# david8862/tf-keras-deeplabv3p-model-set

Measured on AMD Instinct MI355X. Metric: images/sec (513x513, 21-class) MobileNetV2-DeepLabV3+ OS=16 training step, higher is better.
Workload: dtype f32

## Files before the change

### tf-keras-deeplabv3p-model-set_amd/csrc/options.h

```cpp
#pragma once
#include "common.h"

enum OptGet { GET_NONE, GET_SET, GET_LATCHED, GET_LATCHED_GE0, GET_RESOLVED };

#define DL3P_OPTION_TABLE(X)                                                                                                  \
                                                                    \
  X(PW_SMALL_MIN_ROWS, GET_NONE, "pw_small_min_rows", "DL3P_PW_SMALL_MIN_ROWS", 1 << 17, -1, v < 0 ? (1 << 17) : v)           \
                                \
  X(GEMM_NT, GET_NONE, "gemm_nt", nullptr, 0, 0, (v >= 1 && v <= 8) ? v : 0)                                                  \
              \
  X(GEMM_MI, GET_NONE, "gemm_mi", "DL3P_GEMM_MI", 0, 0, (v == 1 || v == 2) ? v : 0)                                           \
  X(GEMM_PER_CU, GET_NONE, "gemm_per_cu", "DL3P_GEMM_PER_CU", 0, 0, v > 0 ? v : 0)                                            \
                                                                \
  X(GEMM_TUNED, GET_NONE, "gemm_tuned", "DL3P_GEMM_TUNED", 1, -1, v ? 1 : 0)                                                  \
                   \
  X(SB_PIPE, GET_RESOLVED, "sb_pipe", "DL3P_SB_PIPE", 0, -1, v ? 1 : 0)                                                       \
                                                        \
  X(SPLIT_WGRAD, GET_LATCHED, "split_wgrad", "DL3P_SPLIT_WGRAD", env_int("DL3P_SPLIT_GEMM", 1), -1, v ? 1 : 0)                \
           \
  X(SPLIT_WGRAD_TILE, GET_NONE, "split_wgrad_tile", nullptr, -1, -1, (v >= 0 && v <= 4) ? v : -1)                             \
  X(SPLIT_WGRAD_PER_CU, GET_NONE, "split_wgrad_per_cu", nullptr, 0, 0, v > 0 ? v : 0)                                         \
                                                        \
  X(SPLITK, GET_SET, "splitk", "DL3P_SPLITK", -1, -1, v)                                                                      \
                     \
  X(SB_WM, GET_NONE, "sb_wm", nullptr, 0, 0, (v >= -1 && v <= 2) ? v : 0)                                                     \
  X(SB_NT, GET_NONE, "sb_nt", nullptr, 0, 0, (v == 8 || v == 12 || v == 16) ? v : 0)                                          \
                                       \
  X(SB_RS, GET_SET, "sb_rs", "DL3P_SB_RS", -1, -1, v < 0 ? -1 : (v ? 1 : 0))                                                  \
                                        \
  X(SB3, GET_LATCHED_GE0, "sb3", "DL3P_SB3", -1, -1, v < 0 ? -1 : (v ? 1 : 0))                                                \
                                     \
  X(BF16_KG, GET_NONE, "bf16_kg", "DL3P_BF16_KG", 0, -1, (v == 0 || v == 1 || v == 2 || v == 4) ? v : -1)                     \
                        \
  X(CONV_SB, GET_SET, "conv_sb", "DL3P_CONV_SB", 1, -1, (v >= 0 && v <= 2) ? v : -1)                                          \
                                      \
  X(DW_PER_CU, GET_NONE, "dw_per_cu", nullptr, 0, 0, v > 0 ? v : 0)                                                           \
  X(DW_WANT, GET_NONE, "dw_want", "DL3P_DW_WANT", DL3P_NUM_CUS * 3 / 2, 0, v > 0 ? v : 0)                                     \
  X(DW_MAXTH, GET_NONE, "dw_maxth", "DL3P_DW_MAXTH", 16, 0, v > 0 ? v : 0)                                                    \
  X(DW_TW, GET_NONE, "dw_tw", nullptr, 0, 0, (v == 2 || v == 4) ? v : 0)                                                      \
  X(DW_TUNED, GET_NONE, "dw_tuned", "DL3P_DW_TUNED", 1, -1, v ? 1 : 0)                                                        \
                                                                                                               \
  X(WGRAD_TILE, GET_NONE, "wgrad_tile", "DL3P_WGRAD_TILE", -1, -1, (v >= 0 && v <= 3) ? v : -1)                               \
  X(WGRAD_PER_CU, GET_NONE, "wgrad_per_cu", "DL3P_WGRAD_PER_CU", 4, 0, v > 0 ? v : 0)

enum Opt {
#define X(id, get, name, env, def, unset, norm) OPT_##id,
  DL3P_OPTION_TABLE(X)
#undef X
  OPT_COUNT
};

struct OptState { int set, env; bool env_read; };
extern OptState g_opt[OPT_COUNT];
int opt_env_read(Opt id);

static constexpr int k_opt_unset[OPT_COUNT] = {
#define X(id, get, name, env, def, unset, norm) unset,
  DL3P_OPTION_TABLE(X)
#undef X
};

static inline int opt_set(Opt id) { return g_opt[id].set; }
static inline int opt_env(Opt id) { return g_opt[id].env_read ? g_opt[id].env : opt_env_read(id); }
static inline int opt(Opt id) { return g_opt[id].set != k_opt_unset[id] ? g_opt[id].set : opt_env(id); }
```

### tf-keras-deeplabv3p-model-set_amd/csrc/pw_gemm_kernels.h

```cpp
#pragma once
#include "pw_gemm.h"
#include <type_traits>

typedef float f32x4 __attribute__((ext_vector_type(4)));

#ifndef DL3P_GEMM_PIN_B
#define DL3P_GEMM_PIN_B 1
#endif
template <int NT, bool B_KN, bool STATS, int MI, int BKT, bool BNB = false, bool GA = false>
__global__ __launch_bounds__(256, 2) void pw_gemm_kernel(GemmParams p_in) {
  GemmParams p = p_in;
  int block_y = blockIdx.y;
#ifndef DL3P_NO_SPLITK
  if constexpr (!B_KN && !STATS && !BNB && !GA) {
    if (p.ksplit > 1) {
      const int nbn = (int)gridDim.y / p.ksplit;
      const int z = block_y / nbn;
      block_y -= z * nbn;
      const int k_lo = z * p.kchunk;
      p.A += k_lo;
      if (p.scale) { p.scale += k_lo; p.shift += k_lo; }
      p.B += k_lo;
      p.K = min(p.kchunk, p.K - k_lo);
      p.Y += (size_t)z * p.M * p.ldy;
// ... 353 lines not shown
    for (int idx = t; idx < KP * NP; idx += 256) {
      const int n = idx / KP, k = idx - n * KP;
      Bs[k * BP + n] = (k < p.K && n < p.N) ? p.B[(size_t)n * p.ldb + k] : 0.f;
    }
  }
  for (int i = t; i < KP; i += 256) {
    sc_s[i] = (p.scale && i < p.K) ? p.scale[i] : 1.f;
    sh_s[i] = (p.scale && i < p.K) ? p.shift[i] : 0.f;
  }
  if (BNB) {
    for (int i = t; i < NP; i += 256) {
      const bool in = i < p.N;
      bq_s[i] = in ? p.bb_scale[i] : 1.f;
      bq_s[NP + i] = in ? p.bb_shift[i] : 0.f;
      bq_s[2 * NP + i] = in ? p.bb_mean[i] : 0.f;
      bq_s[3 * NP + i] = in ? p.bb_invstd[i] : 0.f;
    }
  }
  __syncthreads();

  uint32_t a_k[KT];
  bool a_kok[KT];
#pragma unroll
  for (int kt = 0; kt < KT; ++kt) {
    const int k = kt * 16 + 4 * q;
    a_kok[kt] = k < p.K;
    a_k[kt] = (uint32_t)min(k, p.K - 4) * 4u;
  }
  const int n4 = p.N >> 2, nf = 4 * p.N;
  int yrow[NTN], yl[NTN];
  uint32_t yg[NTN], zg[BNB ? NTN : 1];
#pragma unroll
  for (int i = 0; i < NTN; ++i) {
    const int f = min(l + 64 * i, nf - 1);
    const int r = f / n4, c = f - r * n4;
    yrow[i] = (l + 64 * i < nf) ? r : (1 << 20);
    yl[i] = r * TP + c * 4;
    yg[i] = ((uint32_t)r * (uint32_t)p.ldy + (uint32_t)c * 4u) * 4u;
    if (BNB) zg[i] = ((uint32_t)r * (uint32_t)p.bb_ldz + (uint32_t)c * 4u) * 4u;
  }
  const char* Zb = reinterpret_cast<const char*>(p.bb_z);
  const float act_lo = p.act == DL3P_ACT_NONE ? -DL3P_INF : 0.f;
  const float act_hi = (p.act == DL3P_ACT_NONE || p.act == DL3P_ACT_RELU) ? DL3P_INF : 6.f;

  f32x4 acc[NTN];
#pragma unroll
  for (int b = 0; b < NTN; ++b) acc[b] = (f32x4){0.f, 0.f, 0.f, 0.f};
  float4 st_s[STATS ? NTN : 1], st_q[STATS ? NTN : 1];
  if (STATS) {
#pragma unroll
    for (int i = 0; i < NTN; ++i) { st_s[i] = zero4(); st_q[i] = zero4(); }
  }

  const int ntiles = (p.M + 15) >> 4;
  const int nwaves = gridDim.x * 4;
  const int gw = blockIdx.x * 4 + w;
  const char* Ab = reinterpret_cast<const char*>(p.A);
  char* Yb = reinterpret_cast<char*>(p.Y);
  float4 ra[KT];
#define SM_PREFETCH(tile_)                                                                                   \
  {                                                                                                          \
    const uint32_t arow = (uint32_t)min(((tile_) << 4) + l15, p.M - 1) * (uint32_t)p.lda * 4u;              \
    _Pragma("unroll") for (int kt = 0; kt < KT; ++kt) ra[kt] = *reinterpret_cast<const float4*>(Ab + (arow + a_k[kt])); \
  }
  SM_PREFETCH(min(gw, ntiles - 1))
  for (int tile = gw; tile < ntiles; tile += nwaves) {
    const int m0 = tile << 4;
    const bool row_ok = m0 + l15 < p.M;
    float4 zpre[BNB ? NTN : 1];
    if (BNB) {
      const uint32_t zbase = (uint32_t)m0 * (uint32_t)p.bb_ldz * 4u;
#pragma unroll
      for (int i = 0; i < NTN; ++i) {
        const uint32_t off = (yrow[i] < p.M - m0) ? zg[i] : 0u;
        zpre[i] = *reinterpret_cast<const float4*>(Zb + (zbase + off));
      }
    }
    float4 a[KT];
#pragma unroll
    for (int kt = 0; kt < KT; ++kt) {
      const float4 s4 = *reinterpret_cast<const float4*>(&sc_s[kt * 16 + 4 * q]);
      const float4 h4 = *reinterpret_cast<const float4*>(&sh_s[kt * 16 + 4 * q]);
      float4 v = fma4(ra[kt], s4, h4);
      if (p.act >= DL3P_ACT_HSWISH) v = act_apply4(v, p.act);
      else v = make_float4(__builtin_amdgcn_fmed3f(v.x, act_lo, act_hi), __builtin_amdgcn_fmed3f(v.y, act_lo, act_hi),
                           __builtin_amdgcn_fmed3f(v.z, act_lo, act_hi), __builtin_amdgcn_fmed3f(v.w, act_lo, act_hi));
      a[kt] = (row_ok && a_kok[kt]) ? v : zero4();
    }
    SM_PREFETCH(min(tile + nwaves, ntiles - 1))
#pragma unroll
    for (int kt = 0; kt < KT; ++kt) {
      const float av[4] = {a[kt].x, a[kt].y, a[kt].z, a[kt].w};
#pragma unroll
      for (int nt = 0; nt < NTN; ++nt)
#pragma unroll
        for (int j = 0; j < 4; ++j)
          acc[nt] = __builtin_amdgcn_mfma_f32_16x16x4f32(Bs[(kt * 16 + 4 * q + j) * BP + nt * 16 + l15], av[j], acc[nt], 0, 0, 0);
    }
#pragma unroll
    for (int nt = 0; nt < NTN; ++nt) {
      *reinterpret_cast<float4*>(&Ts[l15 * TP + nt * 16 + 4 * q]) = make_float4(acc[nt][0], acc[nt][1], acc[nt][2], acc[nt][3]);
      acc[nt] = (f32x4){0.f, 0.f, 0.f, 0.f};
    }
    const uint32_t ybase = (uint32_t)m0 * (uint32_t)p.ldy * 4u;
    const int rows_here = p.M - m0;
#pragma unroll
    for (int i = 0; i < NTN; ++i) {
      if (yrow[i] < rows_here) {
        float4 o = *reinterpret_cast<const float4*>(&Ts[yl[i]]);
        if (p.bias) o = add4(o, ld4(p.bias + (yl[i] - yrow[i] * TP)));
        float* yp = reinterpret_cast<float*>(Yb + (ybase + yg[i]));
        if (p.accumulate) o = add4(o, ld4(yp));
#ifdef DL3P_ABLATE_STORES
        if (o.x == 1234.5678f)
#endif
        st4(yp, o);
        if (STATS && BNB) {
          const int cf = yl[i] - yrow[i] * TP;
          const float4 zv = zpre[i];
          const float4 u = fma4(zv, *reinterpret_cast<const float4*>(&bq_s[cf]), *reinterpret_cast<const float4*>(&bq_s[NP + cf]));
          const float4 mu = *reinterpret_cast<const float4*>(&bq_s[2 * NP + cf]), is = *reinterpret_cast<const float4*>(&bq_s[3 * NP + cf]);
          const float4 d = make_float4(o.x * act_grad(u.x, p.bb_act), o.y * act_grad(u.y, p.bb_act),
                                       o.z * act_grad(u.z, p.bb_act), o.w * act_grad(u.w, p.bb_act));
          const float4 xh = make_float4((zv.x - mu.x) * is.x, (zv.y - mu.y) * is.y, (zv.z - mu.z) * is.z, (zv.w - mu.w) * is.w);
          st_s[i] = add4(st_s[i], d);
          st_q[i] = fma4(d, xh, st_q[i]);
        } else if (STATS) {
          st_s[i] = add4(st_s[i], o);
          st_q[i] = fma4(o, o, st_q[i]);
        }
      }
    }
  }
#undef SM_PREFETCH
  if (STATS) {
    float4* S = reinterpret_cast<float4*>(Tall);
#pragma unroll
    for (int which = 0; which < 2; ++which) {
      __syncthreads();
#pragma unroll
      for (int i = 0; i < NTN; ++i)
        if (l + 64 * i < nf) S[w * 4 * NP + l + 64 * i] = which ? st_q[i] : st_s[i];
      __syncthreads();
      if (p.partials && t < n4) {
        float4 s = zero4();
        for (int ww = 0; ww < 4; ++ww)
          for (int r = 0; r < 16; ++r) s = add4(s, S[ww * 4 * NP + r * n4 + t]);
        st4(p.partials + ((size_t)blockIdx.x * 2 + which) * p.N + 4 * t, s);
      }
    }
  }
}

template <int KT, int NTN, bool BNB = false>
static constexpr size_t pw_small_lds() {
  return sizeof(float) * (size_t)(16 * KT * (16 * NTN + 4) + 2 * 16 * KT + (BNB ? 4 * 16 * NTN : 0) + 4 * 16 * (16 * NTN + 4));
}
```

### tf-keras-deeplabv3p-model-set_amd/csrc/pwconv.hip

```cpp
#include "common.h"
#include "options.h"
#include "pw_gemm_kernels.h"
#include "pw_wgrad_kernels.h"
#include <algorithm>

enum GemmForm {
  FORM_PIPE = 0,
  FORM_TILED = 1,
  FORM_WIDE = 2,
  FORM_ROW_STATIONARY = 3,
  FORM_PINNED = 4,
  FORM_STREAMING,
  FORM_TINY
};
struct SmallShape { int kt, ntn; };
struct GemmPlan {
  GemmForm form;
  int nt, mi, wm;
  int gx, gy, m_tiles;
  SmallShape small;
  bool from_table;
};
struct GemmTraits {
  int act = DL3P_ACT_NONE;
// ... 241 lines not shown
  if (opt_set(OPT_GEMM_NT)) pl.nt = opt_set(OPT_GEMM_NT) > 8 ? 8 : opt_set(OPT_GEMM_NT);
  gemm_grid(&pl, M, N, false, opt_set(OPT_GEMM_MI) ? opt_set(OPT_GEMM_MI) : ((M >= 4096 && pl.nt < 6) ? 2 : 1), opt_set(OPT_GEMM_PER_CU));
  return pl;
}

static bool sb3d_takes(int M, int K, int N, int pitch, int bn_act, int front_act, bool bnb, bool accumulate, int ld_max) {
  static const int sb3d = env_int("DL3P_SB3_DGRAD", 0);
  const int sb3 = opt(OPT_SB3);
  if (sb3 == 0 || !dl3p_sb3d_supported(M, K, N, pitch, bn_act, front_act, bnb, accumulate, ld_max)) return false;
  return sb3 == 1 || (sb3d && M >= 65536);
}

extern "C" int dl3p_pwconv_fwd_splitk_plan(int M, int K, int N) {
  const int force = opt_set(OPT_SPLITK);
  if (force == 0 || (force < 0 && opt_env(OPT_SPLITK) == 0)) return 0;
  if (!(N == 128 || N == 256 || N == 512) || K % 4 || K < 512 || M < 1024) return 0;
  if ((unsigned long long)M * (unsigned long long)K * 4ull >= (1ull << 32)) return 0;
  const int tiles = ceil_div(M, 64) * ceil_div(N, 128);
  if (force < 0 && (tiles > 640 || K < 1024)) return 0;
  int S = force > 0 ? force : 5;
  S = std::min(S, std::min(16, K / 256));
  while (S > 1 && ceil_div(ceil_div(K, S), 32) * 32 * (S - 1) >= K) --S;
  return S > 1 ? S : 0;
}
extern "C" size_t dl3p_pwconv_fwd_splitk_workspace(int M, int K, int N) {
  const int S = dl3p_pwconv_fwd_splitk_plan(M, K, N);
  return S ? sizeof(float) * (size_t)S * M * N : 0;
}

enum WgradForm { WGRAD_TILED = 0, WGRAD_STREAMING = 1, WGRAD_TINY = 2, WGRAD_SPLIT = 4 };
struct WgradPlan {
  WgradForm form;
  int slabs;
  bool has_small; SmallShape small; int small_grid;
  int kw, nw, ktiles, ntiles, mchunk, tiled_slabs;
  int pin_per_cu; bool from_table;
  int sb_slabs, kf, sb_nw, sb_ktiles, sb_ntiles, mrows;
};
struct WgradTraits {
  size_t max_slabs = DL3P_MAX_STAT_ROWS;
  bool tiny_ok = true, streaming_ok = true, split_ok = true;
  bool gathered = false;
};

static int wgrad_small_grid(int M, int KT, int NTN) {
  const int tiles = ceil_div(M, 16);
  static const int occ_env = env_int("DL3P_WGRAD_SMALL_PER_CU", 2);
  const int occ = occ_env, tpw = 2;
  (void)KT; (void)NTN;
  int g = tiles / (4 * tpw);
  if (g > DL3P_NUM_CUS * occ) g = DL3P_NUM_CUS * occ;
  if (g > DL3P_MAX_STAT_ROWS) g = DL3P_MAX_STAT_ROWS;
  if (g < 1) g = 1;
  return g;
}

static bool wgrad_small_pick(int K, int N, SmallShape* out) {
  static const SmallShape list[] = {{1, 2}, {2, 1}, {2, 2}, {1, 6}, {2, 3}, {2, 4}, {4, 2}, {6, 2}, {2, 6}, {2, 9}, {9, 2},
                                    {2, 12}, {12, 2}, {4, 4}};
  static const int off = env_int("DL3P_WGRAD_SMALL", 1) == 0;
  if (off) return false;
  const int kt = ceil_div(K, 16), ntn = ceil_div(N, 16);
  int best = -1, best_tiles = 1 << 30;
  for (int i = 0; i < (int)(sizeof(list) / sizeof(list[0])); ++i)
    if (list[i].kt >= kt && list[i].ntn >= ntn && list[i].kt * list[i].ntn < best_tiles) { best = i; best_tiles = list[i].kt * list[i].ntn; }
  if (best < 0 || best_tiles > 2 * kt * ntn) return false;
  *out = list[best];
  return true;
}

static void wgrad_tiled_plan(WgradPlan* pl, int M, int K, int N) {
  static const int cand[4][2] = {{1, 4}, {2, 4}, {1, 8}, {2, 8}};
  const GemmTuned* e = gemm_tuned_lookup(4, M, K, N);
  pl->from_table = e != nullptr;
  int force = opt_env(OPT_WGRAD_TILE);
  if (e) force = e->nt;
  if (opt_set(OPT_WGRAD_TILE) >= 0) force = opt_set(OPT_WGRAD_TILE);
  pl->kw = 1; pl->nw = 4;
  if (force >= 0 || M >= 65536) {
    float best = 1e30f;
    for (int i = 0; i < 4; ++i) {
      if (force >= 0 && i != force) continue;
      const int tk = 64 * cand[i][0], tn = 16 * cand[i][1];
      const float area = (float)(ceil_div(K, tk) * tk) * (float)(ceil_div(N, tn) * tn);
      const float cost = area * (1.f + 0.5f * (64.f / tk + 64.f / tn));
      if (cost < best) { best = cost; pl->kw = cand[i][0]; pl->nw = cand[i][1]; }
    }
  }
  pl->ktiles = ceil_div(K, 64 * pl->kw);
  pl->ntiles = ceil_div(N, 16 * pl->nw);
  const int tiles = pl->ktiles * pl->ntiles;
  int per_cu = opt_env(OPT_WGRAD_PER_CU);
  if (e) per_cu = e->mi;
  if (opt_set(OPT_WGRAD_PER_CU)) per_cu = opt_set(OPT_WGRAD_PER_CU);
  pl->pin_per_cu = opt_set(OPT_WGRAD_PER_CU) ? opt_set(OPT_WGRAD_PER_CU) : (e ? e->mi : 0);
  int s = (DL3P_NUM_CUS * per_cu) / tiles;
  if (s < 1) s = 1;
  int max_s = ceil_div(M, 256);
  if (s > max_s) s = max_s;
  if (s > DL3P_MAX_STAT_ROWS) s = DL3P_MAX_STAT_ROWS;
  int chunk = ceil_div(ceil_div(M, s), 32) * 32;
  pl->tiled_slabs = ceil_div(M, chunk);
  pl->mchunk = chunk;
}

extern "C" int dl3p_conv2d_gemm_sb_pays(int role, int M, int K, int N);
static void wgrad_sb_route(WgradPlan* pl, int M, int K, int N, const WgradTraits& t) {
  int tile = opt_set(OPT_SPLIT_WGRAD_TILE), per_cu = opt_set(OPT_SPLIT_WGRAD_PER_CU);
  if (t.gathered) {
    if (!dl3p_conv2d_gemm_sb_pays(4, M, K, N)) return;
    if (tile == 4) tile = 0;
  } else {
    if (opt(OPT_SPLIT_WGRAD) <= 0) return;
    if (tile < 0 && per_cu <= 0) {
      const int pays = dl3p_pwconv_sb_pays(4, M, K, N);
      if (pays == 0 || (pays < 0 && (K < 128 || N < 128 || M < 16384))) return;
      if (const GemmTuned* e = gemm_tuned_lookup(9, M, K, N)) { tile = e->nt; per_cu = e->mi; }
    }
  }
  const int max_slabs = (int)std::min(t.max_slabs, (size_t)DL3P_MAX_STAT_ROWS);
  pl->sb_slabs = dl3p_wgrad_sb_plan(M, K, N, max_slabs, tile, per_cu, &pl->kf, &pl->sb_nw, &pl->sb_ktiles, &pl->sb_ntiles, &pl->mrows);
}

static WgradPlan plan_wgrad(int M, int K, int N, const WgradTraits& t = WgradTraits()) {
  WgradPlan pl = {};
  wgrad_tiled_plan(&pl, M, K, N);
  pl.has_small = !t.gathered && wgrad_small_pick(K, N, &pl.small);
  if (pl.has_small) pl.small_grid = wgrad_small_grid(M, pl.small.kt, pl.small.ntn);
  if (!t.gathered && t.tiny_ok && dl3p_pw_tiny_applies(M)) { pl.form = WGRAD_TINY; return pl; }
  if (M >= 16 && pl.has_small && t.streaming_ok) { pl.form = WGRAD_STREAMING; pl.slabs = pl.small_grid; return pl; }
  if (t.split_ok) wgrad_sb_route(&pl, M, K, N, t);
  pl.form = pl.sb_slabs > 0 ? WGRAD_SPLIT : WGRAD_TILED;
  pl.slabs = pl.sb_slabs > 0 ? pl.sb_slabs : pl.tiled_slabs;
  return pl;
}
static size_t wgrad_workspace_slabs(int M, int K, int N, bool gathered) {
  WgradTraits t;
  t.tiny_ok = false; t.gathered = gathered;
  const WgradPlan pl = plan_wgrad(M, K, N, t);
  return pl.has_small ? (size_t)pl.small_grid : (size_t)std::max(pl.tiled_slabs, pl.sb_slabs);
}

template <int KT, int NTN, bool STATS, bool BNB = false>
static void launch_pw_small(const GemmParams& p, int grid, hipStream_t st) {
  constexpr size_t lds = pw_small_lds<KT, NTN, BNB>();
  static bool attr_set = false;
  if (!attr_set) {
    (void)hipFuncSetAttribute((const void*)pw_small_kernel<KT, NTN, STATS, BNB>, hipFuncAttributeMaxDynamicSharedMemorySize, (int)lds);
    attr_set = true;
  }
  dl3p_launch(pw_small_kernel<KT, NTN, STATS, BNB>, dim3(grid), dim3(256), lds, st, p);
}

template <bool STATS, bool BNB = false>
static void launch_pw_small_any(const GemmParams& p, SmallShape sh, int grid, hipStream_t st) {
#define DL3P_PS(a, b) if (sh.kt == a && sh.ntn == b) { launch_pw_small<a, b, STATS, BNB>(p, grid, st); return; }
  DL3P_PS(1, 2) DL3P_PS(2, 1) DL3P_PS(6, 1) DL3P_PS(1, 6) DL3P_PS(2, 3) DL3P_PS(3, 2) DL3P_PS(6, 2) DL3P_PS(2, 6)
  DL3P_PS(2, 9) DL3P_PS(9, 2)
#undef DL3P_PS
}

template <int NT, bool B_KN, bool STATS, int MI, int BKT, bool BNB = false, bool GA = false>
static void launch_gemm_one(const GemmParams& p, dim3 grid, hipStream_t st) {
  constexpr int BM = 64 * MI, BN = 16 * NT, AP = BKT + 4;
  constexpr int BS = B_KN ? BKT * (BN + 4) : BN * AP;
  constexpr int TPP = NT < 4 ? NT : 4;
  constexpr int ES = 4 * 16 * MI * (16 * TPP + 4);
  constexpr int OPER = BM * AP + BS;
  constexpr int RED = STATS ? 2 * 4 * BN : 0;
  constexpr size_t lds = sizeof(float) * (size_t)((BKT > 32 ? (OPER > ES ? OPER : ES) : OPER + ES) + RED);
  static bool attr_set = false;
  if (!attr_set) {
    if (lds > 64 * 1024)
      (void)hipFuncSetAttribute((const void*)pw_gemm_kernel<NT, B_KN, STATS, MI, BKT, BNB, GA>, hipFuncAttributeMaxDynamicSharedMemorySize, (int)lds);
    attr_set = true;
  }
  dl3p_launch(pw_gemm_kernel<NT, B_KN, STATS, MI, BKT, BNB, GA>, grid, dim3(256), lds, st, p);
}

template <bool B_KN, bool STATS, int MI, int BKT, bool BNB = false, bool GA = false>
static void launch_gemm_mi(const GemmParams& p, int nt, dim3 grid, hipStream_t st) {
  switch (nt) {
    case 1: launch_gemm_one<1, B_KN, STATS, MI, BKT, BNB, GA>(p, grid, st); break;
    case 2: launch_gemm_one<2, B_KN, STATS, MI, BKT, BNB, GA>(p, grid, st); break;
    case 3: launch_gemm_one<3, B_KN, STATS, MI, BKT, BNB, GA>(p, grid, st); break;
    case 4: launch_gemm_one<4, B_KN, STATS, MI, BKT, BNB, GA>(p, grid, st); break;
    case 5: launch_gemm_one<5, B_KN, STATS, MI, BKT, BNB, GA>(p, grid, st); break;
    case 6: launch_gemm_one<6, B_KN, STATS, MI, BKT, BNB, GA>(p, grid, st); break;
    case 7: launch_gemm_one<7, B_KN, STATS, MI, BKT, BNB, GA>(p, grid, st); break;
    default: launch_gemm_one<8, B_KN, STATS, MI, BKT, BNB, GA>(p, grid, st); break;
  }
}

template <bool B_KN, bool STATS, bool BNB = false, bool GA = false>
static void launch_gemm(const GemmParams& p_in, int nt, int mi, dim3 grid, hipStream_t st) {
  GemmParams p = p_in;
  if (mi == 1) launch_gemm_mi<B_KN, STATS, 1, 32, BNB, GA>(p, nt, grid, st);
  else launch_gemm_mi<B_KN, STATS, 2, 32, BNB, GA>(p, nt, grid, st);
}

template <int KT, int NTN, bool BNA = false>
static void launch_wgrad_small(const WgradParams& p, int grid, hipStream_t st) {
  constexpr size_t lds = wgrad_small_lds<KT, NTN, BNA>();
  static bool attr_set = false;
  if (!attr_set) {
    (void)hipFuncSetAttribute((const void*)pw_wgrad_small_kernel<KT, NTN, BNA>, hipFuncAttributeMaxDynamicSharedMemorySize, (int)lds);
    attr_set = true;
  }
  dl3p_launch(pw_wgrad_small_kernel<KT, NTN, BNA>, dim3(grid), dim3(256), lds, st, p);
}

template <bool BNA = false>
static void launch_wgrad_small_any(const WgradParams& p, SmallShape sh, int grid, hipStream_t st) {
#define DL3P_WS(a, b) if (sh.kt == a && sh.ntn == b) { launch_wgrad_small<a, b, BNA>(p, grid, st); return; }
  DL3P_WS(1, 2) DL3P_WS(2, 1) DL3P_WS(2, 2) DL3P_WS(1, 6) DL3P_WS(2, 3) DL3P_WS(2, 4) DL3P_WS(4, 2) DL3P_WS(6, 2)
  DL3P_WS(2, 6) DL3P_WS(2, 9) DL3P_WS(9, 2) DL3P_WS(2, 12) DL3P_WS(12, 2) DL3P_WS(4, 4)
#undef DL3P_WS
}

template <bool GX = false, bool BNA = false>
static void launch_wgrad_tiled(const WgradParams& p, const WgradPlan& pl, hipStream_t st) {
  const int kw = pl.kw, nw = pl.nw;
  const dim3 grid(p.ktiles * p.ntiles, pl.tiled_slabs), block(256);
  if (kw == 1 && nw == 4) dl3p_launch(pw_wgrad_kernel<1, 4, GX, BNA>, grid, block, 0, st, p);
  else if (kw == 2 && nw == 4) dl3p_launch(pw_wgrad_kernel<2, 4, GX, BNA>, grid, block, 0, st, p);
  else if (kw == 1 && nw == 8) dl3p_launch(pw_wgrad_kernel<1, 8, GX, BNA>, grid, block, 0, st, p);
  else dl3p_launch(pw_wgrad_kernel<2, 8, GX, BNA>, grid, block, 0, st, p);
}

static int launch_plan_sb(const char* fn, const GemmParams& p, const GemmPlan& pl, bool stats, bool bnb, hipStream_t st) {
  switch (pl.form) {
    case FORM_PINNED:
      DL3P_CHECK_ARG(dl3p_launch_gemm_sb3(p, stats, pl.gx, st), "%s: no pinned-schedule instantiation for activation %d", fn, p.act);
      break;
    case FORM_ROW_STATIONARY:
      DL3P_CHECK_ARG(dl3p_launch_gemm_sbr(p, bnb ? 2 : (stats ? 1 : 0), pl.gx, st), "%s: no row-stationary instantiation for K=%d", fn, p.K);
      break;
    case FORM_PIPE: dl3p_launch_gemm_sbp(p, stats, bnb, pl.nt, pl.mi, dim3(pl.gx, pl.gy), st); break;
    default: dl3p_launch_gemm_sb(p, stats, bnb, false, pl.nt, pl.mi, pl.wm, dim3(pl.gx, pl.gy), st); break;
  }
  DL3P_CHECK_LAUNCH(fn);
  return DL3P_OK;
}

__global__ __launch_bounds__(256) void splitk_finish_kernel(const float* __restrict__ slabs, int S, const float* __restrict__ bias,
                                                            float* __restrict__ y, int ldy, float* __restrict__ partials, int M,
                                                            int N, int rows_per_wg) {
  __shared__ float red[2][256 * 4];
  const int c4n = N / 4;
  const int rpp = 256 / c4n;
  const int c4 = threadIdx.x % c4n, rg = threadIdx.x / c4n;
  const int r0 = blockIdx.x * rows_per_wg;
  float4 s = zero4(), ss = zero4();
  float4 b4 = zero4();
  if (bias) b4 = ld4(bias + c4 * 4);
  for (int r = r0 + rg; r < min(r0 + rows_per_wg, M); r += rpp) {
    float4 acc = ld4(slabs + ((size_t)r * N + c4 * 4));
    for (int z = 1; z < S; ++z) acc = add4(acc, ld4(slabs + (((size_t)z * M + r) * N + c4 * 4)));
    acc = add4(acc, b4);
    st4(y + (size_t)r * ldy + c4 * 4, acc);
    s = add4(s, acc);
    ss.x = fmaf(acc.x, acc.x, ss.x); ss.y = fmaf(acc.y, acc.y, ss.y); ss.z = fmaf(acc.z, acc.z, ss.z); ss.w = fmaf(acc.w, acc.w, ss.w);
  }
  if (!partials) return;
  *reinterpret_cast<float4*>(&red[0][threadIdx.x * 4]) = s;
  *reinterpret_cast<float4*>(&red[1][threadIdx.x * 4]) = ss;
  __syncthreads();
  if (rg == 0) {
    float4 a = zero4(), b = zero4();
    for (int g = 0; g < rpp; ++g) {
      a = add4(a, *reinterpret_cast<const float4*>(&red[0][(g * c4n + c4) * 4]));
      b = add4(b, *reinterpret_cast<const float4*>(&red[1][(g * c4n + c4) * 4]));
    }
    st4(partials + ((size_t)blockIdx.x * 2) * N + c4 * 4, a);
    st4(partials + ((size_t)blockIdx.x * 2 + 1) * N + c4 * 4, b);
  }
}

__global__ __launch_bounds__(256) void transpose_batch_kernel(const float* src, float* dst, const int* table) {
  __shared__ float tile[64][65];
  const int off = table[blockIdx.x * 4], K = table[blockIdx.x * 4 + 1], N = table[blockIdx.x * 4 + 2];
  const int tx = threadIdx.x & 63, ty = threadIdx.x >> 6;
  const int tk = (K + 63) / 64, tn = (N + 63) / 64;
  for (int tl = blockIdx.y; tl < tk * tn; tl += gridDim.y) {
    const int k0 = (tl / tn) * 64, n0 = (tl % tn) * 64;
    float v[16];
    const int n = n0 + tx, nc = n < N ? n : N - 1;
#pragma unroll
    for (int i = 0; i < 16; ++i) {
      const int k = k0 + ty + 4 * i;
      v[i] = src[off + (size_t)(k < K ? k : K - 1) * N + nc];
    }
    __syncthreads();
#pragma unroll
    for (int i = 0; i < 16; ++i) tile[ty + 4 * i][tx] = v[i];
    __syncthreads();
#pragma unroll
    for (int i = 0; i < 16; ++i) {
      const int nn = n0 + ty + 4 * i, k = k0 + tx;
      if (k < K && nn < N) dst[off + (size_t)nn * K + k] = tile[tx][ty + 4 * i];
    }
  }
}

__global__ __launch_bounds__(256) void colsum_kernel(const float* dy, int lddy, long long M, int C, int c4s, int px,
                                                     int nbx, float* partials) {
  const int b = blockIdx.x;
  const int slab = b / nbx;
  const int bx = b - slab * nbx;
// ... 691 lines not shown
```

Baseline: 1365.

## Add software-pipelined small pointwise GEMM kernel with compile-time epilogue variants

Adds a new small-shape pointwise GEMM kernel that double-buffers the A-tile register loads (and the BN z / accumulate-Y loads) one or two tiles ahead. The MFMA work of the current tile then overlaps the global loads for the next, with sched_barriers to keep the order. Bias and accumulate epilogues become template parameters, so runtime branches drop out of the inner loop. The path is on by default through a new option, except for the KT=9, NTN=2 non-BNB shape, and falls back to the old kernel for unsupported epilogues. The extra register sets raise VGPR pressure, which may lower occupancy.

After: 1369, median of 5. About the same (+0.2%).

```diff
diff --git a/tf-keras-deeplabv3p-model-set_amd/csrc/options.h b/tf-keras-deeplabv3p-model-set_amd/csrc/options.h
--- a/tf-keras-deeplabv3p-model-set_amd/csrc/options.h
+++ b/tf-keras-deeplabv3p-model-set_amd/csrc/options.h
@@ -41,7 +41,9 @@
   X(DW_TUNED, GET_NONE, "dw_tuned", "DL3P_DW_TUNED", 1, -1, v ? 1 : 0)                                                        \
                                                                                                                \
   X(WGRAD_TILE, GET_NONE, "wgrad_tile", "DL3P_WGRAD_TILE", -1, -1, (v >= 0 && v <= 3) ? v : -1)                               \
-  X(WGRAD_PER_CU, GET_NONE, "wgrad_per_cu", "DL3P_WGRAD_PER_CU", 4, 0, v > 0 ? v : 0)
+  X(WGRAD_PER_CU, GET_NONE, "wgrad_per_cu", "DL3P_WGRAD_PER_CU", 4, 0, v > 0 ? v : 0)                                         \
+                                                  \
+  X(PW_SMALL_PIPE, GET_NONE, "pw_small_pipe", "DL3P_PW_SMALL_PIPE", 1, -1, v < 0 ? -1 : (v > 1 ? 2 : v))
 
 enum Opt {
 #define X(id, get, name, env, def, unset, norm) OPT_##id,
diff --git a/tf-keras-deeplabv3p-model-set_amd/csrc/pw_gemm_kernels.h b/tf-keras-deeplabv3p-model-set_amd/csrc/pw_gemm_kernels.h
--- a/tf-keras-deeplabv3p-model-set_amd/csrc/pw_gemm_kernels.h
+++ b/tf-keras-deeplabv3p-model-set_amd/csrc/pw_gemm_kernels.h
@@ -529,6 +529,249 @@
   }
 }
 
+template <int KT, int NTN, bool STATS, bool BNB = false, int EPI = 0>
+__global__ __launch_bounds__(256, 2) void pw_small_pipe_kernel(GemmParams p) {
+  constexpr bool BIAS = (EPI & 1) != 0, ACC = (EPI & 2) != 0;
+  constexpr bool ZY_AHEAD = NTN * ((BNB ? 1 : 0) + (ACC ? 1 : 0)) <= 4;
+  constexpr bool TWO_SETS = !(BNB && NTN >= 9);
+  constexpr int KP = 16 * KT, NP = 16 * NTN;
+  constexpr int BP = NP + 4, TP = NP + 4;
+  extern __shared__ __attribute__((aligned(16))) float sm_lds[];
+  float* Bs = sm_lds;
+  float* sc_s = Bs + KP * BP;
+  float* sh_s = sc_s + KP;
+  float* bq_s = sh_s + KP;
+  float* Tall = bq_s + (BNB ? 4 * NP : 0);
+  const int t = threadIdx.x, l = t & 63, w = t >> 6, l15 = l & 15, q = l >> 4;
+  float* Ts = Tall + w * 16 * TP;
+  if (p.b_kn) {
+    for (int idx = t; idx < KP * NP; idx += 256) {
+      const int k = idx / NP, n = idx - k * NP;
+      Bs[k * BP + n] = (k < p.K && n < p.N) ? p.B[(size_t)k * p.ldb + n] : 0.f;
+    }
+  } else {
+    for (int idx = t; idx < KP * NP; idx += 256) {
+      const int n = idx / KP, k = idx - n * KP;
+      Bs[k * BP + n] = (k < p.K && n < p.N) ? p.B[(size_t)n * p.ldb + k] : 0.f;
+    }
+  }
+  for (int i = t; i < KP; i += 256) {
+    sc_s[i] = (p.scale && i < p.K) ? p.scale[i] : 1.f;
+    sh_s[i] = (p.scale && i < p.K) ? p.shift[i] : 0.f;
+  }
+  if (BNB) {
+    for (int i = t; i < NP; i += 256) {
+      const bool in = i < p.N;
+      bq_s[i] = in ? p.bb_scale[i] : 1.f;
+      bq_s[NP + i] = in ? p.bb_shift[i] : 0.f;
+      bq_s[2 * NP + i] = in ? p.bb_mean[i] : 0.f;
+      bq_s[3 * NP + i] = in ? p.bb_invstd[i] : 0.f;
+    }
+  }
+  __syncthreads();
+
+  uint32_t a_k[KT];
+  bool a_kok[KT];
+#pragma unroll
+  for (int kt = 0; kt < KT; ++kt) {
+    const int k = kt * 16 + 4 * q;
+    a_kok[kt] = k < p.K;
+    a_k[kt] = (uint32_t)min(k, p.K - 4) * 4u;
+  }
+  const int n4 = p.N >> 2, nf = 4 * p.N;
+  uint32_t yrc[NTN];
+#pragma unroll
+  for (int i = 0; i < NTN; ++i) {
+    const int f = min(l + 64 * i, nf - 1);
+    const int r = f / n4, c = f - r * n4;
+    yrc[i] = ((uint32_t)r << 16) | ((uint32_t)c * 16u);
+  }
+  const uint32_t ldy4 = (uint32_t)p.ldy * 4u, ldz4 = BNB ? (uint32_t)p.bb_ldz * 4u : 0u;
+#define SP_ITEM(i_)                                                                                          \
+  uint32_t rc_ = yrc[i_];                                                                                    \
+  asm volatile("" : "+v"(rc_));                                                                              \
+  const uint32_t yr_ = rc_ >> 16, cfb_ = rc_ & 0xffffu;                                                      \
+  const float* tsp_ = reinterpret_cast<const float*>(reinterpret_cast<const char*>(Ts) + __umul24(yr_, TP * 4u) + cfb_); \
+  const uint32_t yg_ = __umul24(yr_, ldy4) + cfb_;                                                           \
+  const uint32_t zg_ = __umul24(yr_, ldz4) + cfb_;                                                           \
+  (void)zg_; (void)yg_; (void)tsp_;
+  const char* Zb = reinterpret_cast<const char*>(p.bb_z);
+  const float act_lo = p.act == DL3P_ACT_NONE ? -DL3P_INF : 0.f;
+  const float act_hi = (p.act == DL3P_ACT_NONE || p.act == DL3P_ACT_RELU) ? DL3P_INF : 6.f;
+  float4 bias_r[BIAS ? NTN : 1];
+  if (BIAS) {
+#pragma unroll
+    for (int i = 0; i < NTN; ++i) bias_r[i] = ld4(p.bias + ((yrc[i] & 0xffffu) >> 2));
+  }
+
+  f32x4 acc[NTN];
+#pragma unroll
+  for (int b = 0; b < NTN; ++b) acc[b] = (f32x4){0.f, 0.f, 0.f, 0.f};
+  float4 st_s[STATS ? NTN : 1], st_q[STATS ? NTN : 1];
+  if (STATS) {
+#pragma unroll
+    for (int i = 0; i < NTN; ++i) { st_s[i] = zero4(); st_q[i] = zero4(); }
+  }
+
+  const int nfull = p.M >> 4;
+  const int nwaves = gridDim.x * 4;
+  const int gw = blockIdx.x * 4 + w;
+  const char* Ab = reinterpret_cast<const char*>(p.A);
+  char* Yb = reinterpret_cast<char*>(p.Y);
+
+#define SP_APPLY(dst_, src_, ok_)                                                                            \
+  _Pragma("unroll") for (int kt = 0; kt < KT; ++kt) {                                                        \
+    const float4 s4 = *reinterpret_cast<const float4*>(&sc_s[kt * 16 + 4 * q]);                              \
+    const float4 h4 = *reinterpret_cast<const float4*>(&sh_s[kt * 16 + 4 * q]);                              \
+    float4 v = fma4(src_[kt], s4, h4);                                                                       \
+    if (p.act >= DL3P_ACT_HSWISH) v = act_apply4(v, p.act);                                                  \
+    else v = make_float4(__builtin_amdgcn_fmed3f(v.x, act_lo, act_hi), __builtin_amdgcn_fmed3f(v.y, act_lo, act_hi), \
+                         __builtin_amdgcn_fmed3f(v.z, act_lo, act_hi), __builtin_amdgcn_fmed3f(v.w, act_lo, act_hi)); \
+    dst_[kt] = ((ok_) && a_kok[kt]) ? v : zero4();                                                           \
+  }
+#define SP_MFMA(a_)                                                                                          \
+  _Pragma("unroll") for (int kt = 0; kt < KT; ++kt) {                                                        \
+    const float av[4] = {a_[kt].x, a_[kt].y, a_[kt].z, a_[kt].w};                                            \
+    _Pragma("unroll") for (int nt = 0; nt < NTN; ++nt)                                                       \
+      _Pragma("unroll") for (int j = 0; j < 4; ++j)                                                          \
+        acc[nt] = __builtin_amdgcn_mfma_f32_16x16x4f32(Bs[(kt * 16 + 4 * q + j) * BP + nt * 16 + l15], av[j], acc[nt], 0, 0, 0); \
+  }                                                                                                          \
+  _Pragma("unroll") for (int nt = 0; nt < NTN; ++nt) {                                                       \
+    *reinterpret_cast<float4*>(&Ts[l15 * TP + nt * 16 + 4 * q]) = make_float4(acc[nt][0], acc[nt][1], acc[nt][2], acc[nt][3]); \
+    acc[nt] = (f32x4){0.f, 0.f, 0.f, 0.f};                                                                   \
+  }
+#define SP_STATS(i_, o_, zv_)                                                                                \
+  if constexpr (STATS && BNB) {                                                                              \
+    const int cf = (int)(cfb_ >> 2);                                                                         \
+    const float4 zv = zv_;                                                                                   \
+    const float4 u = fma4(zv, *reinterpret_cast<const float4*>(&bq_s[cf]), *reinterpret_cast<const float4*>(&bq_s[NP + cf])); \
+    const float4 mu = *reinterpret_cast<const float4*>(&bq_s[2 * NP + cf]), is = *reinterpret_cast<const float4*>(&bq_s[3 * NP + cf]); \
+    const float4 d = make_float4(o_.x * act_grad(u.x, p.bb_act), o_.y * act_grad(u.y, p.bb_act),             \
+                                 o_.z * act_grad(u.z, p.bb_act), o_.w * act_grad(u.w, p.bb_act));            \
+    const float4 xh = make_float4((zv.x - mu.x) * is.x, (zv.y - mu.y) * is.y, (zv.z - mu.z) * is.z, (zv.w - mu.w) * is.w); \
+    st_s[i_] = add4(st_s[i_], d);                                                                            \
+    st_q[i_] = fma4(d, xh, st_q[i_]);                                                                        \
+  } else if constexpr (STATS) {                                                                              \
+    st_s[i_] = add4(st_s[i_], o_);                                                                           \
+    st_q[i_] = fma4(o_, o_, st_q[i_]);                                                                       \
+  }
+
+  if (gw < nfull) {
+    float4 ra[TWO_SETS ? 2 : 1][KT], rz[ZY_AHEAD ? 2 : 1][BNB ? NTN : 1], ry[ZY_AHEAD ? 2 : 1][ACC ? NTN : 1];
+#define SP_LOAD_A(S_, tile_)                                                                                 \
+  {                                                                                                          \
+    const uint32_t arow = (uint32_t)((min((tile_), nfull - 1) << 4) + l15) * (uint32_t)p.lda * 4u;           \
+    _Pragma("unroll") for (int kt = 0; kt < KT; ++kt) ra[S_][kt] = *reinterpret_cast<const float4*>(Ab + (arow + a_k[kt])); \
+  }
+#define SP_LOAD_ZY(S_, tile_)                                                                                \
+  {                                                                                                          \
+    const uint32_t pm0 = (uint32_t)(min((tile_), nfull - 1) << 4);                                           \
+    if constexpr (BNB) {                                                                                     \
+      const uint32_t zbase = pm0 * (uint32_t)p.bb_ldz * 4u;                                                  \
+      _Pragma("unroll") for (int i = 0; i < NTN; ++i) { SP_ITEM(i) rz[S_][i] = *reinterpret_cast<const float4*>(Zb + (zbase + zg_)); } \
+    }                                                                                                        \
+    if constexpr (ACC) {                                                                                     \
+      const uint32_t ybase = pm0 * (uint32_t)p.ldy * 4u;                                                     \
+      _Pragma("unroll") for (int i = 0; i < NTN; ++i) { SP_ITEM(i) ry[S_][i] = *reinterpret_cast<const float4*>(Yb + (ybase + yg_)); } \
+    }                                                                                                        \
+  }
+#define SP_TILE(S_, tile_, D_)                                                                                \
+  {                                                                                                          \
+    float4 a[KT];                                                                                            \
+    SP_APPLY(a, ra[S_], true)                                                                                \
+    if constexpr (!ZY_AHEAD) SP_LOAD_ZY(0, (tile_))                                                          \
+    SP_LOAD_A(S_, (tile_) + (D_) * nwaves)                                                                   \
+    if constexpr (ZY_AHEAD) SP_LOAD_ZY(1 - S_, (tile_) + nwaves)                                             \
+    __builtin_amdgcn_sched_barrier(0);                                                                       \
+    SP_MFMA(a)                                                                                               \
+    const uint32_t ybase = (uint32_t)((tile_) << 4) * (uint32_t)p.ldy * 4u;                                  \
+    _Pragma("unroll") for (int i = 0; i < NTN; ++i) {                                                        \
+      SP_ITEM(i)                                                                                             \
+      float4 o = *reinterpret_cast<const float4*>(tsp_);                                                     \
+      if constexpr (BIAS) o = add4(o, bias_r[i]);                                                            \
+      if constexpr (ACC) o = add4(o, ry[ZY_AHEAD ? S_ : 0][i]);                                              \
+      st4(reinterpret_cast<float*>(Yb + (ybase + yg_)), o);                                                  \
+      SP_STATS(i, o, rz[BNB && ZY_AHEAD ? S_ : 0][BNB ? i : 0])                                              \
+                                                      \
+      if constexpr (BNB) __builtin_amdgcn_sched_barrier(0);                                                  \
+    }                                                                                                        \
+    __builtin_amdgcn_sched_barrier(0);                                                                       \
+  }
+    SP_LOAD_A(0, gw)
+    if constexpr (TWO_SETS) SP_LOAD_A(1, gw + nwaves)
+    if constexpr (ZY_AHEAD) SP_LOAD_ZY(0, gw)
+    __builtin_amdgcn_s_waitcnt(0x0F70);
+    if constexpr (TWO_SETS) {
+      int tile = gw;
+      for (; tile + nwaves < nfull; tile += 2 * nwaves) {
+        SP_TILE(0, tile, 2)
+        SP_TILE(1, tile + nwaves, 2)
+      }
+      if (tile < nfull) SP_TILE(0, tile, 2)
+    } else {
+      static_assert(TWO_SETS || !ZY_AHEAD, "one A set goes with one z / output set");
+      for (int tile = gw; tile < nfull; tile += nwaves) SP_TILE(0, tile, 1)
+    }
+#undef SP_TILE
+#undef SP_LOAD_ZY
+#undef SP_LOAD_A
+  }
+  if ((p.M & 15) && gw == nfull % nwaves) {
+    const int m0 = nfull << 4, rows_here = p.M - m0;
+    const bool row_ok = l15 < rows_here;
+    float4 ra[KT], a[KT];
+    const uint32_t arow = (uint32_t)min(m0 + l15, p.M - 1) * (uint32_t)p.lda * 4u;
+#pragma unroll
+    for (int kt = 0; kt < KT; ++kt) ra[kt] = *reinterpret_cast<const float4*>(Ab + (arow + a_k[kt]));
+    float4 zpre[BNB ? NTN : 1];
+    if (BNB) {
+      const uint32_t zbase = (uint32_t)m0 * (uint32_t)p.bb_ldz * 4u;
+#pragma unroll
+      for (int i = 0; i < NTN; ++i) {
+        SP_ITEM(i)
+        const uint32_t off = ((int)yr_ < rows_here) ? zg_ : 0u;
+        zpre[i] = *reinterpret_cast<const float4*>(Zb + (zbase + off));
+      }
+    }
+    SP_APPLY(a, ra, row_ok)
+    SP_MFMA(a)
+    const uint32_t ybase = (uint32_t)m0 * (uint32_t)p.ldy * 4u;
+#pragma unroll
+    for (int i = 0; i < NTN; ++i) {
+      SP_ITEM(i)
+      if (l + 64 * i < nf && (int)yr_ < rows_here) {
+        float4 o = *reinterpret_cast<const float4*>(tsp_);
+        if (BIAS) o = add4(o, bias_r[i]);
+        float* yp = reinterpret_cast<float*>(Yb + (ybase + yg_));
+        if (ACC) o = add4(o, ld4(yp));
+        st4(yp, o);
+        SP_STATS(i, o, zpre[BNB ? i : 0])
+      }
+    }
+  }
+#undef SP_STATS
+#undef SP_ITEM
+#undef SP_MFMA
+#undef SP_APPLY
+  if (STATS) {
+    float4* S = reinterpret_cast<float4*>(Tall);
+#pragma unroll
+    for (int which = 0; which < 2; ++which) {
+      __syncthreads();
+#pragma unroll
+      for (int i = 0; i < NTN; ++i)
+        if (l + 64 * i < nf) S[w * 4 * NP + l + 64 * i] = which ? st_q[i] : st_s[i];
+      __syncthreads();
+      if (p.partials && t < n4) {
+        float4 s = zero4();
+        for (int ww = 0; ww < 4; ++ww)
+          for (int r = 0; r < 16; ++r) s = add4(s, S[ww * 4 * NP + r * n4 + t]);
+        st4(p.partials + ((size_t)blockIdx.x * 2 + which) * p.N + 4 * t, s);
+      }
+    }
+  }
+}
+
 template <int KT, int NTN, bool BNB = false>
 static constexpr size_t pw_small_lds() {
   return sizeof(float) * (size_t)(16 * KT * (16 * NTN + 4) + 2 * 16 * KT + (BNB ? 4 * 16 * NTN : 0) + 4 * 16 * (16 * NTN + 4));
diff --git a/tf-keras-deeplabv3p-model-set_amd/csrc/pwconv.hip b/tf-keras-deeplabv3p-model-set_amd/csrc/pwconv.hip
--- a/tf-keras-deeplabv3p-model-set_amd/csrc/pwconv.hip
+++ b/tf-keras-deeplabv3p-model-set_amd/csrc/pwconv.hip
@@ -417,9 +417,40 @@
   dl3p_launch(pw_small_kernel<KT, NTN, STATS, BNB>, dim3(grid), dim3(256), lds, st, p);
 }
 
+template <int KT, int NTN, bool STATS, bool BNB, int EPI>
+static void launch_pw_small_pipe(const GemmParams& p, int grid, hipStream_t st) {
+  constexpr size_t lds = pw_small_lds<KT, NTN, BNB>();
+  static bool attr_set = false;
+  if (!attr_set) {
+    (void)hipFuncSetAttribute((const void*)pw_small_pipe_kernel<KT, NTN, STATS, BNB, EPI>, hipFuncAttributeMaxDynamicSharedMemorySize, (int)lds);
+    attr_set = true;
+  }
+  dl3p_launch(pw_small_pipe_kernel<KT, NTN, STATS, BNB, EPI>, dim3(grid), dim3(256), lds, st, p);
+}
+template <int KT, int NTN, bool STATS, bool BNB>
+static bool launch_pw_small_pipe_epi(const GemmParams& p, int grid, hipStream_t st) {
+  const int epi = (p.bias ? 1 : 0) | (p.accumulate ? 2 : 0);
+  if (epi == 0) { launch_pw_small_pipe<KT, NTN, STATS, BNB, 0>(p, grid, st); return true; }
+  if (epi == 2) { launch_pw_small_pipe<KT, NTN, STATS, BNB, 2>(p, grid, st); return true; }
+  if constexpr (!STATS && !BNB) {
+    if (epi == 1) { launch_pw_small_pipe<KT, NTN, STATS, BNB, 1>(p, grid, st); return true; }
+  }
+  return false;
+}
+
+template <bool BNB>
+static bool pw_small_pipe_pays(int kt, int ntn) { return BNB || !(kt == 9 && ntn == 2); }
+
 template <bool STATS, bool BNB = false>
 static void launch_pw_small_any(const GemmParams& p, SmallShape sh, int grid, hipStream_t st) {
-#define DL3P_PS(a, b) if (sh.kt == a && sh.ntn == b) { launch_pw_small<a, b, STATS, BNB>(p, grid, st); return; }
+  const int mode = opt(OPT_PW_SMALL_PIPE);
+  const bool pipe = mode > 1 || (mode == 1 && pw_small_pipe_pays<BNB>(sh.kt, sh.ntn));
+#define DL3P_PS(a, b)                                                                          \
+  if (sh.kt == a && sh.ntn == b) {                                                             \
+    if (pipe && launch_pw_small_pipe_epi<a, b, STATS, BNB>(p, grid, st)) return;               \
+    launch_pw_small<a, b, STATS, BNB>(p, grid, st);                                            \
+    return;                                                                                    \
+  }
   DL3P_PS(1, 2) DL3P_PS(2, 1) DL3P_PS(6, 1) DL3P_PS(1, 6) DL3P_PS(2, 3) DL3P_PS(3, 2) DL3P_PS(6, 2) DL3P_PS(2, 6)
   DL3P_PS(2, 9) DL3P_PS(9, 2)
 #undef DL3P_PS
```
